# PaddlePaddle/PaddleNLP

Hardware: NVIDIA H100
Metric: tokens/sec Llama-3.2-3B seq4096 bf16 pretrain step (global, all GPUs) (higher is better)
Workload: dtype bf16

## Files before the change

paddlenlp_b200/csrc/abi.cu:

```cuda
#include <string.h>

#include <mutex>

#include "../../include/b200nlp.h"
#include "common.cuh"
#include "host_util.h"

namespace b200 {

static thread_local char tls_err[512] = "";

void set_last_error(const char* fmt, ...) {
  va_list ap;
  va_start(ap, fmt);
  vsnprintf(tls_err, sizeof(tls_err), fmt, ap);
  va_end(ap);
}
int fail_arg(const char* fmt, ...) {
  va_list ap;
  va_start(ap, fmt);
  vsnprintf(tls_err, sizeof(tls_err), fmt, ap);
  va_end(ap);
  return -1;
}
// ... 24 lines not shown
    cached[dev] = n > 0 ? n : 132;
  }
  return cached[dev];
}

typedef CUresult (*EncodeTiledFn)(CUtensorMap*, CUtensorMapDataType, cuuint32_t, void*, const cuuint64_t*,
                                  const cuuint64_t*, const cuuint32_t*, const cuuint32_t*, CUtensorMapInterleave,
                                  CUtensorMapSwizzle, CUtensorMapL2promotion, CUtensorMapFloatOOBfill);

static EncodeTiledFn get_encode_fn() {
  static EncodeTiledFn fn = nullptr;
  static std::once_flag once;
  std::call_once(once, []() {
    void* p = nullptr;
    cudaDriverEntryPointQueryResult qres;
    cudaError_t e = cudaGetDriverEntryPoint("cuTensorMapEncodeTiled", &p, cudaEnableDefault, &qres);
    if (e == cudaSuccess && qres == cudaDriverEntryPointSuccess) fn = reinterpret_cast<EncodeTiledFn>(p);
  });
  return fn;
}

static int encode_tmap(CUtensorMap* out, CUtensorMapDataType dtype, const void* base, int rank, const uint64_t* dims,
                       const uint64_t* strides, const uint32_t* box);

int encode_tmap_bf16(CUtensorMap* out, const void* base, int rank, const uint64_t* dims, const uint64_t* strides,
                     const uint32_t* box) {
  return encode_tmap(out, CU_TENSOR_MAP_DATA_TYPE_BFLOAT16, base, rank, dims, strides, box);
}
int encode_tmap_f32(CUtensorMap* out, const void* base, int rank, const uint64_t* dims, const uint64_t* strides,
                    const uint32_t* box) {
  return encode_tmap(out, CU_TENSOR_MAP_DATA_TYPE_FLOAT32, base, rank, dims, strides, box);
}

static int encode_tmap(CUtensorMap* out, CUtensorMapDataType dtype, const void* base, int rank, const uint64_t* dims,
                       const uint64_t* strides, const uint32_t* box) {
  EncodeTiledFn fn = get_encode_fn();
  if (!fn) return fail_arg("cuTensorMapEncodeTiled entry point unavailable (no CUDA driver?)");
  cuuint64_t gdim[5];
  cuuint64_t gstr[5];
  cuuint32_t bdim[5];
  cuuint32_t estr[5];
  for (int i = 0; i < rank; ++i) {
    gdim[i] = dims[i];
    bdim[i] = box[i];
    estr[i] = 1;
    if (i < rank - 1) gstr[i] = strides[i];
  }
  if ((reinterpret_cast<uintptr_t>(base) & 15) != 0) return fail_arg("tensor map base %p not 16-byte aligned", base);
  for (int i = 0; i < rank - 1; ++i)
    if (gstr[i] % 16 != 0) return fail_arg("tensor map stride %llu not a multiple of 16 bytes", (unsigned long long)gstr[i]);
  CUresult r = fn(out, dtype, static_cast<cuuint32_t>(rank), const_cast<void*>(base), gdim,
                  gstr, bdim, estr, CU_TENSOR_MAP_INTERLEAVE_NONE, CU_TENSOR_MAP_SWIZZLE_128B,
                  CU_TENSOR_MAP_L2_PROMOTION_L2_256B, CU_TENSOR_MAP_FLOAT_OOB_FILL_NONE);
  if (r != CUDA_SUCCESS)
    return fail_arg("cuTensorMapEncodeTiled failed (CUresult %d) rank=%d dims=[%llu,%llu] box=[%u,%u]", (int)r, rank,
                    (unsigned long long)dims[0], (unsigned long long)(rank > 1 ? dims[1] : 0), box[0],
                    rank > 1 ? box[1] : 0);
  return 0;
}

}

extern "C" {

const char* b200_last_error(void) { return b200::tls_err; }

// ... 36 lines not shown
```

paddlenlp_b200/csrc/common.cuh:

```cuda
#pragma once
#include <cuda.h>
#include <cuda_bf16.h>
#include <cuda_runtime.h>
#include <stdint.h>
#include <stdio.h>

namespace b200 {

typedef __nv_bfloat16 bf16;

__device__ __forceinline__ uint32_t smem_u32(const void* p) {
  return static_cast<uint32_t>(__cvta_generic_to_shared(p));
}
__device__ __forceinline__ void named_bar_sync(uint32_t id, uint32_t nthreads) {
  asm volatile("bar.sync %0, %1;" ::"r"(id), "r"(nthreads) : "memory");
}

__device__ __forceinline__ void pdl_wait() { asm volatile("griddepcontrol.wait;" ::: "memory"); }
__device__ __forceinline__ void pdl_launch_dependents() { asm volatile("griddepcontrol.launch_dependents;" ::: "memory"); }

__device__ __forceinline__ void mbar_init(uint64_t* bar, uint32_t count) {
  asm volatile("mbarrier.init.shared::cta.b64 [%0], %1;" ::"r"(smem_u32(bar)), "r"(count) : "memory");
}
__device__ __forceinline__ void fence_mbar_init() {
  asm volatile("fence.mbarrier_init.release.cluster;" ::: "memory");
}
__device__ __forceinline__ void fence_proxy_async_smem() {
  asm volatile("fence.proxy.async.shared::cta;" ::: "memory");
}
__device__ __forceinline__ void mbar_arrive_expect_tx(uint64_t* bar, uint32_t bytes) {
  asm volatile("mbarrier.arrive.expect_tx.shared::cta.b64 _, [%0], %1;" ::"r"(smem_u32(bar)), "r"(bytes)
               : "memory");
}
__device__ __forceinline__ void mbar_arrive(uint64_t* bar) {
  asm volatile("mbarrier.arrive.shared::cta.b64 _, [%0];" ::"r"(smem_u32(bar)) : "memory");
}
__device__ __forceinline__ bool mbar_try_wait(uint64_t* bar, uint32_t parity) {
  uint32_t ok;
  asm volatile(
      "{\n\t.reg .pred P;\n\t"
      "mbarrier.try_wait.parity.shared::cta.b64 P, [%1], %2;\n\t"
      "selp.u32 %0, 1, 0, P;\n\t}\n"
      : "=r"(ok)
      : "r"(smem_u32(bar)), "r"(parity)
      : "memory");
  return ok != 0;
}
__device__ __forceinline__ void mbar_wait(uint64_t* bar, uint32_t parity) {
// ... 60 lines not shown
  uint64_t d = 0;
  d |= static_cast<uint64_t>((saddr & 0x3FFFFu) >> 4);
  d |= static_cast<uint64_t>((lbo_bytes >> 4) & 0x3FFFu) << 16;
  d |= static_cast<uint64_t>((sbo_bytes >> 4) & 0x3FFFu) << 32;
  d |= static_cast<uint64_t>(1) << 62;
  return d;
}
__device__ __forceinline__ void wgmma_fence() { asm volatile("wgmma.fence.sync.aligned;" ::: "memory"); }
__device__ __forceinline__ void wgmma_commit() { asm volatile("wgmma.commit_group.sync.aligned;" ::: "memory"); }
template <int N>
__device__ __forceinline__ void wgmma_wait() { asm volatile("wgmma.wait_group.sync.aligned %0;" ::"n"(N) : "memory"); }
template <int R>
__device__ __forceinline__ void setmaxnreg_dec() { asm volatile("setmaxnreg.dec.sync.aligned.u32 %0;" ::"n"(R)); }
template <int R>
__device__ __forceinline__ void setmaxnreg_inc() { asm volatile("setmaxnreg.inc.sync.aligned.u32 %0;" ::"n"(R)); }

template <int TA, int TB>
__device__ __forceinline__ void wgmma_m64n256k16(float (&d)[128], uint64_t desc_a, uint64_t desc_b, uint32_t accumulate) {
  asm volatile(
      "{\n\t.reg .pred p;\n\tsetp.ne.b32 p, %130, 0;\n\t"
      "wgmma.mma_async.sync.aligned.m64n256k16.f32.bf16.bf16 "
      "{%0, %1, %2, %3, %4, %5, %6, %7, %8, %9, %10, %11, %12, %13, %14, %15, %16, %17, %18, %19, %20, %21, %22, %23, %24, %25, %26, %27, %28, %29, %30, %31, %32, %33, %34, %35, %36, %37, %38, %39, %40, %41, %42, %43, %44, %45, %46, %47, %48, %49, %50, %51, %52, %53, %54, %55, %56, %57, %58, %59, %60, %61, %62, %63, %64, %65, %66, %67, %68, %69, %70, %71, %72, %73, %74, %75, %76, %77, %78, %79, %80, %81, %82, %83, %84, %85, %86, %87, %88, %89, %90, %91, %92, %93, %94, %95, %96, %97, %98, %99, %100, %101, %102, %103, %104, %105, %106, %107, %108, %109, %110, %111, %112, %113, %114, %115, %116, %117, %118, %119, %120, %121, %122, %123, %124, %125, %126, %127}, %128, %129, p, 1, 1, %131, %132;\n\t}\n"
      : "+f"(d[0]), "+f"(d[1]), "+f"(d[2]), "+f"(d[3]), "+f"(d[4]), "+f"(d[5]), "+f"(d[6]), "+f"(d[7]), "+f"(d[8]), "+f"(d[9]), "+f"(d[10]), "+f"(d[11]), "+f"(d[12]), "+f"(d[13]), "+f"(d[14]), "+f"(d[15]), "+f"(d[16]), "+f"(d[17]), "+f"(d[18]), "+f"(d[19]), "+f"(d[20]), "+f"(d[21]), "+f"(d[22]), "+f"(d[23]), "+f"(d[24]), "+f"(d[25]), "+f"(d[26]), "+f"(d[27]), "+f"(d[28]), "+f"(d[29]), "+f"(d[30]), "+f"(d[31]), "+f"(d[32]), "+f"(d[33]), "+f"(d[34]), "+f"(d[35]), "+f"(d[36]), "+f"(d[37]), "+f"(d[38]), "+f"(d[39]), "+f"(d[40]), "+f"(d[41]), "+f"(d[42]), "+f"(d[43]), "+f"(d[44]), "+f"(d[45]), "+f"(d[46]), "+f"(d[47]), "+f"(d[48]), "+f"(d[49]), "+f"(d[50]), "+f"(d[51]), "+f"(d[52]), "+f"(d[53]), "+f"(d[54]), "+f"(d[55]), "+f"(d[56]), "+f"(d[57]), "+f"(d[58]), "+f"(d[59]), "+f"(d[60]), "+f"(d[61]), "+f"(d[62]), "+f"(d[63]), "+f"(d[64]), "+f"(d[65]), "+f"(d[66]), "+f"(d[67]), "+f"(d[68]), "+f"(d[69]), "+f"(d[70]), "+f"(d[71]), "+f"(d[72]), "+f"(d[73]), "+f"(d[74]), "+f"(d[75]), "+f"(d[76]), "+f"(d[77]), "+f"(d[78]), "+f"(d[79]), "+f"(d[80]), "+f"(d[81]), "+f"(d[82]), "+f"(d[83]), "+f"(d[84]), "+f"(d[85]), "+f"(d[86]), "+f"(d[87]), "+f"(d[88]), "+f"(d[89]), "+f"(d[90]), "+f"(d[91]), "+f"(d[92]), "+f"(d[93]), "+f"(d[94]), "+f"(d[95]), "+f"(d[96]), "+f"(d[97]), "+f"(d[98]), "+f"(d[99]), "+f"(d[100]), "+f"(d[101]), "+f"(d[102]), "+f"(d[103]), "+f"(d[104]), "+f"(d[105]), "+f"(d[106]), "+f"(d[107]), "+f"(d[108]), "+f"(d[109]), "+f"(d[110]), "+f"(d[111]), "+f"(d[112]), "+f"(d[113]), "+f"(d[114]), "+f"(d[115]), "+f"(d[116]), "+f"(d[117]), "+f"(d[118]), "+f"(d[119]), "+f"(d[120]), "+f"(d[121]), "+f"(d[122]), "+f"(d[123]), "+f"(d[124]), "+f"(d[125]), "+f"(d[126]), "+f"(d[127])
      : "l"(desc_a), "l"(desc_b), "r"(accumulate), "n"(TA), "n"(TB));
}
template <int TA, int TB>
__device__ __forceinline__ void wgmma_m64n64k16(float (&d)[32], uint64_t desc_a, uint64_t desc_b, uint32_t accumulate) {
  asm volatile(
      "{\n\t.reg .pred p;\n\tsetp.ne.b32 p, %34, 0;\n\t"
      "wgmma.mma_async.sync.aligned.m64n64k16.f32.bf16.bf16 "
      "{%0, %1, %2, %3, %4, %5, %6, %7, %8, %9, %10, %11, %12, %13, %14, %15, %16, %17, %18, %19, %20, %21, %22, %23, %24, %25, %26, %27, %28, %29, %30, %31}, %32, %33, p, 1, 1, %35, %36;\n\t}\n"
      : "+f"(d[0]), "+f"(d[1]), "+f"(d[2]), "+f"(d[3]), "+f"(d[4]), "+f"(d[5]), "+f"(d[6]), "+f"(d[7]), "+f"(d[8]), "+f"(d[9]), "+f"(d[10]), "+f"(d[11]), "+f"(d[12]), "+f"(d[13]), "+f"(d[14]), "+f"(d[15]), "+f"(d[16]), "+f"(d[17]), "+f"(d[18]), "+f"(d[19]), "+f"(d[20]), "+f"(d[21]), "+f"(d[22]), "+f"(d[23]), "+f"(d[24]), "+f"(d[25]), "+f"(d[26]), "+f"(d[27]), "+f"(d[28]), "+f"(d[29]), "+f"(d[30]), "+f"(d[31])
      : "l"(desc_a), "l"(desc_b), "r"(accumulate), "n"(TA), "n"(TB));
}
template <int TB>
__device__ __forceinline__ void wgmma_m64n128k16_rs(float (&d)[64], const uint32_t* a, uint64_t desc_b, uint32_t accumulate) {
  asm volatile(
      "{\n\t.reg .pred p;\n\tsetp.ne.b32 p, %69, 0;\n\t"
      "wgmma.mma_async.sync.aligned.m64n128k16.f32.bf16.bf16 "
      "{%0, %1, %2, %3, %4, %5, %6, %7, %8, %9, %10, %11, %12, %13, %14, %15, %16, %17, %18, %19, %20, %21, %22, %23, %24, %25, %26, %27, %28, %29, %30, %31, %32, %33, %34, %35, %36, %37, %38, %39, %40, %41, %42, %43, %44, %45, %46, %47, %48, %49, %50, %51, %52, %53, %54, %55, %56, %57, %58, %59, %60, %61, %62, %63}, {%64, %65, %66, %67}, %68, p, 1, 1, %70;\n\t}\n"
      : "+f"(d[0]), "+f"(d[1]), "+f"(d[2]), "+f"(d[3]), "+f"(d[4]), "+f"(d[5]), "+f"(d[6]), "+f"(d[7]), "+f"(d[8]), "+f"(d[9]), "+f"(d[10]), "+f"(d[11]), "+f"(d[12]), "+f"(d[13]), "+f"(d[14]), "+f"(d[15]), "+f"(d[16]), "+f"(d[17]), "+f"(d[18]), "+f"(d[19]), "+f"(d[20]), "+f"(d[21]), "+f"(d[22]), "+f"(d[23]), "+f"(d[24]), "+f"(d[25]), "+f"(d[26]), "+f"(d[27]), "+f"(d[28]), "+f"(d[29]), "+f"(d[30]), "+f"(d[31]), "+f"(d[32]), "+f"(d[33]), "+f"(d[34]), "+f"(d[35]), "+f"(d[36]), "+f"(d[37]), "+f"(d[38]), "+f"(d[39]), "+f"(d[40]), "+f"(d[41]), "+f"(d[42]), "+f"(d[43]), "+f"(d[44]), "+f"(d[45]), "+f"(d[46]), "+f"(d[47]), "+f"(d[48]), "+f"(d[49]), "+f"(d[50]), "+f"(d[51]), "+f"(d[52]), "+f"(d[53]), "+f"(d[54]), "+f"(d[55]), "+f"(d[56]), "+f"(d[57]), "+f"(d[58]), "+f"(d[59]), "+f"(d[60]), "+f"(d[61]), "+f"(d[62]), "+f"(d[63])
      : "r"(a[0]), "r"(a[1]), "r"(a[2]), "r"(a[3]), "l"(desc_b), "r"(accumulate), "n"(TB));
}

__device__ __forceinline__ void mma_bf16_16816(float (&c)[4], const uint32_t (&a)[4], uint32_t b0, uint32_t b1) {
  asm volatile(
      "mma.sync.aligned.m16n8k16.row.col.f32.bf16.bf16.f32 {%0, %1, %2, %3}, {%4, %5, %6, %7}, {%8, %9}, "
      "{%0, %1, %2, %3};"
      : "+f"(c[0]), "+f"(c[1]), "+f"(c[2]), "+f"(c[3])
      : "r"(a[0]), "r"(a[1]), "r"(a[2]), "r"(a[3]), "r"(b0), "r"(b1));
}
__device__ __forceinline__ void ldsm_x4(uint32_t saddr, uint32_t (&r)[4]) {
  asm volatile("ldmatrix.sync.aligned.m8n8.x4.shared.b16 {%0, %1, %2, %3}, [%4];"
               : "=r"(r[0]), "=r"(r[1]), "=r"(r[2]), "=r"(r[3])
               : "r"(saddr));
}
__device__ __forceinline__ void ldsm_x4_t(uint32_t saddr, uint32_t (&r)[4]) {
  asm volatile("ldmatrix.sync.aligned.m8n8.x4.trans.shared.b16 {%0, %1, %2, %3}, [%4];"
               : "=r"(r[0]), "=r"(r[1]), "=r"(r[2]), "=r"(r[3])
               : "r"(saddr));
}
__device__ __forceinline__ void cp_async_16(uint32_t saddr, const void* gptr, uint32_t src_bytes) {
  asm volatile("cp.async.cg.shared.global [%0], [%1], 16, %2;" ::"r"(saddr), "l"(gptr), "r"(src_bytes) : "memory");
}
__device__ __forceinline__ void cp_async_commit() { asm volatile("cp.async.commit_group;" ::: "memory"); }
template <int N>
// ... 80 lines not shown
```

paddlenlp_b200/csrc/fa_bwd.cu:

```cuda
#include <climits>

#include "../../include/b200nlp.h"
#include "common.cuh"
#include "host_util.h"

namespace b200 {
namespace fab {

constexpr int D = 128;
constexpr int BKV = 64;
constexpr int NUM_THREADS = 256;

struct Params {
  const bf16 *q, *k, *v, *dout;
  int64_t ldq, ldk, ldv, lddo;
  int S, B, nh, kvh, Spad;
  float scale, scale_log2;
  const float* lse2;
  const float* delta;
  const int* mask_start;
  float* dq_acc;
  float* dk_acc;
  float* dv_acc;
};
// ... 214 lines not shown
    o.z = pack_bf16x2(b.x, b.y); o.w = pack_bf16x2(b.z, b.w);
    *(reinterpret_cast<uint4*>(dq + t * lddq) + c) = o;
  }
}

namespace wg {
constexpr int BKV = 128;
constexpr int BQ = 64;
constexpr int STAGES = 2;
constexpr int NUM_THREADS = 256;
constexpr int KV_BYTES = BKV * D * 2;
constexpr int QT_BYTES = BQ * D * 2;
constexpr int STAGE_BYTES = 2 * QT_BYTES + 2 * BQ * 4;
constexpr int STAGE_STRIDE = 33 * 1024;
constexpr int DS_BYTES = BKV * BQ * 2;
constexpr int DQ_BYTES = BQ * 64 * 4;
constexpr int OFF_K = 0, OFF_V = KV_BYTES, OFF_RING = 2 * KV_BYTES;
constexpr int OFF_DS = OFF_RING + STAGES * STAGE_STRIDE;
constexpr int OFF_DQ = OFF_DS + 2 * DS_BYTES;
constexpr int OFF_BAR = OFF_DQ + 2 * DQ_BYTES;
constexpr int SMEM_BYTES = OFF_BAR + 64 + 1024;
static_assert(SMEM_BYTES <= 227 * 1024, "fa_bwd_wgmma: shared memory");
static_assert(STAGE_BYTES <= STAGE_STRIDE && 64 * D * 4 <= STAGE_STRIDE && 64 * D * 4 <= 2 * DS_BYTES && 64 * D * 4 <= 2 * DQ_BYTES,
              "fa_bwd_wgmma: shared-memory layout");

struct Params {
  int S, nh, kvh, Spad;
  float scale, scale_log2;
  const float* lse2;
  const float* delta;
  const int* mask_start;
};

template <int N>
__device__ __forceinline__ void reg_fence(float (&r)[N]) {
#pragma unroll
  for (int i = 0; i < N; ++i) asm volatile("" : "+f"(r[i])::"memory");
}

template <int NJ>
__device__ __forceinline__ void stage_f32(uint32_t base, const float (&acc)[4 * NJ], int wi, int lane) {
  const int g = lane >> 2, tq = lane & 3;
#pragma unroll
  for (int i = 0; i < 2; ++i) {
    const int row = wi * 16 + g + 8 * i;
#pragma unroll
    for (int j = 0; j < NJ; ++j) {
      const int chunk = (j & 3) * 2 + (tq >> 1);
      const uint32_t a = base + (j >> 2) * (64 * 128) + row * 128 + ((chunk ^ (row & 7)) << 4) + (tq & 1) * 8;
      asm volatile("st.shared.v2.f32 [%0], {%1, %2};" ::"r"(a), "f"(acc[4 * j + 2 * i]), "f"(acc[4 * j + 2 * i + 1]) : "memory");
    }
  }
}

template <bool MASK>
__global__ void __launch_bounds__(NUM_THREADS, 1)
fa_bwd_wgmma_kernel(const __grid_constant__ CUtensorMap tmQ, const __grid_constant__ CUtensorMap tmK,
                    const __grid_constant__ CUtensorMap tmV, const __grid_constant__ CUtensorMap tmdO,
                    const __grid_constant__ CUtensorMap tmdQ, const __grid_constant__ CUtensorMap tmdK,
                    const __grid_constant__ CUtensorMap tmdV, const Params p) {
  extern __shared__ uint8_t smem_raw[];
  uint8_t* smem = reinterpret_cast<uint8_t*>((reinterpret_cast<uintptr_t>(smem_raw) + 1023) & ~uintptr_t(1023));
  uint64_t* full_bar = reinterpret_cast<uint64_t*>(smem + OFF_BAR);
  uint64_t* empty_bar = full_bar + STAGES;
  uint64_t* kv_bar = empty_bar + STAGES;

  const int head = static_cast<int>(blockIdx.x) % p.nh, batch = static_cast<int>(blockIdx.x) / p.nh;
  const int kv_head = head / (p.nh / p.kvh);
  const int kv0 = static_cast<int>(blockIdx.y) * BKV;
  int q_lo = kv0 / BQ, q_hi = (p.S + BQ - 1) / BQ;
  if constexpr (MASK) {
    const int last = __ldg(p.mask_start + static_cast<size_t>(batch) * p.S + min(kv0 + BKV - 1, p.S - 1));
// ... 144 lines not shown
    mbar_arrive(&empty_bar[st]);
    uint8_t* sdq = smem + OFF_DQ + cw * DQ_BYTES;
    if (leader) tma_store_wait_read<0>();
    named_bar_sync(2 + cw, 128);
    stage_f32<8>(smem_u32(sdq), dq, wi, lane);
    fence_proxy_async_smem();
    named_bar_sync(2 + cw, 128);
    if (leader) {
      tma_reduce_add_4d(&tmdQ, sdq, cw * 64, head, q0, batch);
      tma_reduce_add_4d(&tmdQ, sdq + DQ_BYTES / 2, cw * 64 + 32, head, q0, batch);
      tma_store_commit();
    }
  }

  if (leader) tma_store_wait_read<0>();
  named_bar_sync(1, 256);
  uint8_t* sdk = smem + OFF_RING + cw * STAGE_STRIDE;
  uint8_t* sdv = smem + (cw == 0 ? OFF_DS : OFF_DQ);
  stage_f32<16>(smem_u32(sdk), dk, wi, lane);
  stage_f32<16>(smem_u32(sdv), dv, wi, lane);
  fence_proxy_async_smem();
  named_bar_sync(2 + cw, 128);
  if (leader) {
#pragma unroll
    for (int b = 0; b < 4; ++b) {
      tma_reduce_add_4d(&tmdK, sdk + b * (64 * 128), b * 32, kv_head, kv0 + cw * 64, batch);
      tma_reduce_add_4d(&tmdV, sdv + b * (64 * 128), b * 32, kv_head, kv0 + cw * 64, batch);
    }
    tma_store_commit();
    tma_store_wait<0>();
  }
}

static int make_bf16_map(CUtensorMap* tm, const void* base, int64_t B, int64_t S, int64_t heads, int64_t ld, uint32_t rows) {
  const uint64_t dims[4] = {128, static_cast<uint64_t>(heads), static_cast<uint64_t>(S), static_cast<uint64_t>(B)};
  const uint64_t strides[3] = {256, static_cast<uint64_t>(ld) * 2, static_cast<uint64_t>(S * ld) * 2};
  const uint32_t box[4] = {64, 1, rows, 1};
  return encode_tmap_bf16(tm, base, 4, dims, strides, box);
}
static int make_f32_map(CUtensorMap* tm, float* base, int64_t B, int64_t S, int64_t heads) {
  const uint64_t dims[4] = {128, static_cast<uint64_t>(heads), static_cast<uint64_t>(S), static_cast<uint64_t>(B)};
  const uint64_t strides[3] = {512, static_cast<uint64_t>(heads) * 512, static_cast<uint64_t>(S * heads) * 512};
  const uint32_t box[4] = {32, 1, 64, 1};
  return encode_tmap_f32(tm, base, 4, dims, strides, box);
}

template <bool MASK>
static int launch(const CUtensorMap (&tm)[7], const Params& p, int B, cudaStream_t stream) {
  auto kern = fa_bwd_wgmma_kernel<MASK>;
  static bool attr_set = false;
  if (!attr_set) {
    cudaError_t e = cudaFuncSetAttribute(kern, cudaFuncAttributeMaxDynamicSharedMemorySize, SMEM_BYTES);
    if (e != cudaSuccess) {
      set_last_error("fa_bwd_wgmma smem attr: %s", cudaGetErrorString(e));
      return static_cast<int>(e);
    }
    attr_set = true;
  }
  const dim3 grid(static_cast<unsigned>(p.nh * B), static_cast<unsigned>((p.S + BKV - 1) / BKV));
  kern<<<grid, NUM_THREADS, SMEM_BYTES, stream>>>(tm[0], tm[1], tm[2], tm[3], tm[4], tm[5], tm[6], p);
  return check_launch("fa_bwd_wgmma");
}
}

template <int BQ, bool MASK>
static int launch(const Params& p, cudaStream_t stream) {
  constexpr int SMEM = 2 * BKV * 256 + 2 * BQ * 256 + 2 * BQ * 128 + 2 * BQ * 4;
  static bool attr_set = false;
  if (!attr_set) {
    cudaError_t e = cudaFuncSetAttribute(fa_bwd_kernel<BQ, MASK>, cudaFuncAttributeMaxDynamicSharedMemorySize, SMEM);
    if (e != cudaSuccess) {
      set_last_error("fa_bwd smem attr: %s", cudaGetErrorString(e));
// ... 47 lines not shown
  float* dk_acc = dq_acc + B * S * num_heads * 128;
  float* dv_acc = dk_acc + B * S * num_kv_heads * 128;
  float* lse2 = dq_acc + 3 * B * S * num_heads * 128;
  float* delta = lse2 + B * num_heads * Spad;
  cudaError_t e = cudaMemsetAsync(dq_acc, 0, static_cast<size_t>(B) * S * (num_heads + 2 * num_kv_heads) * 128 * 4, stream);
  if (e != cudaSuccess) {
    set_last_error("fa_bwd memset: %s", cudaGetErrorString(e));
    return static_cast<int>(e);
  }
  {
    const int64_t rows = B * Spad * num_heads;
    const int64_t threads = rows * 16;
    fa_bwd_delta_kernel<<<static_cast<unsigned>((threads + 255) / 256), 256, 0, stream>>>(
        static_cast<const bf16*>(o), static_cast<const bf16*>(dout), lse, lse2, delta, (int)B, (int)S, (int)Spad, (int)num_heads,
        ldo, lddo);
    int rc = check_launch("fa_bwd(delta)");
    if (rc) return rc;
  }
  int rc;
  if (fa_bwd_impl() == 1) {
    Params p;
    p.q = static_cast<const bf16*>(q); p.k = static_cast<const bf16*>(k); p.v = static_cast<const bf16*>(v);
    p.dout = static_cast<const bf16*>(dout);
    p.ldq = ldq; p.ldk = ldk; p.ldv = ldv; p.lddo = lddo;
    p.S = (int)S; p.B = (int)B; p.nh = (int)num_heads; p.kvh = (int)num_kv_heads; p.Spad = (int)Spad;
    p.scale = softmax_scale;
    p.scale_log2 = softmax_scale * 1.4426950408889634f;
    p.lse2 = lse2; p.delta = delta;
    p.mask_start = mask_start_rows;
    p.dq_acc = dq_acc; p.dk_acc = dk_acc; p.dv_acc = dv_acc;
    rc = mask_start_rows ? launch<64, true>(p, stream) : launch<64, false>(p, stream);
  } else {
    CUtensorMap tm[7];
    if ((rc = wg::make_bf16_map(&tm[0], q, B, S, num_heads, ldq, wg::BQ)) != 0) return rc;
    if ((rc = wg::make_bf16_map(&tm[1], k, B, S, num_kv_heads, ldk, wg::BKV)) != 0) return rc;
    if ((rc = wg::make_bf16_map(&tm[2], v, B, S, num_kv_heads, ldv, wg::BKV)) != 0) return rc;
    if ((rc = wg::make_bf16_map(&tm[3], dout, B, S, num_heads, lddo, wg::BQ)) != 0) return rc;
    if ((rc = wg::make_f32_map(&tm[4], dq_acc, B, S, num_heads)) != 0) return rc;
    if ((rc = wg::make_f32_map(&tm[5], dk_acc, B, S, num_kv_heads)) != 0) return rc;
    if ((rc = wg::make_f32_map(&tm[6], dv_acc, B, S, num_kv_heads)) != 0) return rc;
    wg::Params p;
    p.S = (int)S; p.nh = (int)num_heads; p.kvh = (int)num_kv_heads; p.Spad = (int)Spad;
    p.scale = softmax_scale;
    p.scale_log2 = softmax_scale * 1.4426950408889634f;
    p.lse2 = lse2; p.delta = delta;
    p.mask_start = mask_start_rows;
    rc = mask_start_rows ? wg::launch<true>(tm, p, (int)B, stream) : wg::launch<false>(tm, p, (int)B, stream);
  }
  if (rc) return rc;
  {
    const int64_t tokens = B * S;
    const int width = static_cast<int>(num_heads * 128);
    const int64_t total = tokens * (width / 8);
    int64_t blocks = (total + 255) / 256;
    const int64_t cap = static_cast<int64_t>(sm_count()) * 16;
    if (blocks > cap) blocks = cap;
    fa_bwd_dq_finish_kernel<<<static_cast<unsigned>(blocks), 256, 0, stream>>>(dq_acc, static_cast<bf16*>(dq), tokens,
                                                                              width, lddq);
    if ((rc = check_launch("fa_bwd(dq finish)")) != 0) return rc;
    const int kvw = static_cast<int>(num_kv_heads * 128);
    int64_t kblocks = (tokens * (kvw / 8) + 255) / 256;
    if (kblocks > cap) kblocks = cap;
    fa_bwd_dq_finish_kernel<<<static_cast<unsigned>(kblocks), 256, 0, stream>>>(dk_acc, static_cast<bf16*>(dk), tokens, kvw,
                                                                               lddk);
    if ((rc = check_launch("fa_bwd(dk finish)")) != 0) return rc;
    fa_bwd_dq_finish_kernel<<<static_cast<unsigned>(kblocks), 256, 0, stream>>>(dv_acc, static_cast<bf16*>(dv), tokens, kvw,
                                                                               lddv);
    rc = check_launch("fa_bwd(dv finish)");
  }
  return rc;
// ... 2 lines not shown
```

paddlenlp_b200/csrc/fa_fwd.cu:

```cuda
#include "../../include/b200nlp.h"
#include "common.cuh"
#include "host_util.h"

namespace b200 {
namespace fa {

constexpr int D = 128;
constexpr int BKV = 64;
constexpr int KV_TILE_BYTES = BKV * D * 2;

enum Mode { DENSE = 0, MASK = 1, PAGED = 2 };

struct Params {
  const bf16* q;
  const bf16* k;
  const bf16* v;
  bf16* o;
  float* lse;
  int64_t ldq, ldk, ldv, ldo;
  int S, B, nh, kvh;
  float scale_log2;
  const int* mask_start;
  const int* cu_q;
  const int* seq_dec;
  const int* seq_this;
  const int* seq_enc;
  const int* block_tables;
  int max_blocks, block_size;
};

__device__ __forceinline__ uint32_t swz(int row, int chunk) { return static_cast<uint32_t>(row * 256 + ((chunk ^ (row & 7)) << 4)); }

template <int NW, int MODE>
__global__ void __launch_bounds__(NW * 32, 1) fa_fwd_kernel(const Params p) {
  constexpr int BQ = 16 * NW;
  extern __shared__ __align__(128) uint8_t smem[];
  const uint32_t sQ = smem_u32(smem);
  const uint32_t sK = sQ + BQ * 256;
  const uint32_t sV = sK + 2 * KV_TILE_BYTES;

  const int warp = threadIdx.x >> 5, lane = threadIdx.x & 31;
  const int head = blockIdx.y, batch = blockIdx.z;
  const int kv_head = head / (p.nh / p.kvh);
  int n_rows = p.S, pos0 = 0, tok0 = batch * p.S;
  if constexpr (MODE == PAGED) {
    n_rows = p.seq_this[batch];
    if (n_rows <= 0 || (n_rows == 1 && p.seq_enc[batch] <= 0)) return;
    pos0 = p.seq_dec[batch];
    tok0 = p.cu_q[batch];
  }
  const int qt = (n_rows + BQ - 1) / BQ - 1 - static_cast<int>(blockIdx.x);
  if (qt < 0) return;
  const int q0 = qt * BQ;
  const int kv_total = pos0 + n_rows;
  const int kv_end = pos0 + min(q0 + BQ, n_rows);
  const int n_kv = (kv_end + BKV - 1) / BKV;
  int j_lo = 0;
  if constexpr (MODE == MASK) {
    const int* ms = p.mask_start + static_cast<size_t>(batch) * p.S;
    while (j_lo < n_kv - 1 && __ldg(ms + min(j_lo * BKV + BKV - 1, p.S - 1)) <= q0) ++j_lo;
  }

  auto kv_row = [&](const bf16* base, int64_t ld, int c) -> const bf16* {
    if constexpr (MODE == PAGED) {
      const int page = __ldg(p.block_tables + static_cast<size_t>(batch) * p.max_blocks + c / p.block_size);
      return base + ((static_cast<size_t>(page) * p.kvh + kv_head) * p.block_size + c % p.block_size) * D;
// ... 95 lines not shown
#pragma unroll
      for (int dt = 0; dt < 16; ++dt) { o[dt][2 * h] *= corr; o[dt][2 * h + 1] *= corr; }
    }
#pragma unroll
    for (int kc = 0; kc < 4; ++kc) {
#pragma unroll
      for (int dp = 0; dp < 8; ++dp) {
        uint32_t b[4];
        ldsm_x4_t(vb + swz(kc * 16 + (lane & 7) + ((lane >> 3) & 1) * 8, dp * 2 + (lane >> 4)), b);
        mma_bf16_16816(o[2 * dp], pa[kc], b[0], b[1]);
        mma_bf16_16816(o[2 * dp + 1], pa[kc], b[2], b[3]);
      }
    }
    __syncthreads();
  }
#pragma unroll
  for (int h = 0; h < 2; ++h) {
    float lt = l[h];
    lt += __shfl_xor_sync(0xffffffffu, lt, 1);
    lt += __shfl_xor_sync(0xffffffffu, lt, 2);
    const int r = row_a + 8 * h;
    if (r >= n_rows) continue;
    const float inv = 1.f / lt;
    bf16* orow = p.o + static_cast<size_t>(tok0 + r) * p.ldo + head * D;
#pragma unroll
    for (int dt = 0; dt < 16; ++dt)
      *reinterpret_cast<uint32_t*>(orow + dt * 8 + 2 * tq) = pack_bf16x2(o[dt][2 * h] * inv, o[dt][2 * h + 1] * inv);
    if constexpr (MODE != PAGED) {
      if (tq == 0) p.lse[(static_cast<size_t>(batch) * p.nh + head) * p.S + r] = (m[h] + log2f(lt)) * 0.6931471805599453f;
    }
  }
}

template <int NW, int MODE>
static int launch(const Params& p, int q_rows, cudaStream_t stream) {
  constexpr int SMEM = 16 * NW * 256 + 4 * KV_TILE_BYTES;
  static bool attr_set = false;
  if (!attr_set) {
    cudaError_t e = cudaFuncSetAttribute(fa_fwd_kernel<NW, MODE>, cudaFuncAttributeMaxDynamicSharedMemorySize, SMEM);
    if (e != cudaSuccess) {
      set_last_error("fa_fwd smem attr: %s", cudaGetErrorString(e));
      return static_cast<int>(e);
    }
    attr_set = true;
  }
  dim3 grid(static_cast<unsigned>((q_rows + 16 * NW - 1) / (16 * NW)), static_cast<unsigned>(p.nh), static_cast<unsigned>(p.B));
  fa_fwd_kernel<NW, MODE><<<grid, NW * 32, SMEM, stream>>>(p);
  return check_launch("fa_fwd");
}

}

int launch_fa_prefill_paged(const void* qkv, const void* key_cache, const void* value_cache, void* out, const int32_t* cu_seqlens_q,
                            const int32_t* seq_lens_encoder, const int32_t* seq_lens_decoder, const int32_t* seq_lens_this_time,
                            const int32_t* block_tables, int64_t B, int64_t token_num, int64_t max_q_len, int64_t num_heads,
                            int64_t num_kv_heads, int64_t num_blocks, int64_t block_size, int64_t max_blocks_per_seq, int64_t ldq,
                            int64_t ldo, float softmax_scale, cudaStream_t stream) {
  using namespace fa;
  (void)token_num; (void)num_blocks;
  Params p = {};
  p.q = static_cast<const bf16*>(qkv);
  p.k = static_cast<const bf16*>(key_cache);
  p.v = static_cast<const bf16*>(value_cache);
  p.o = static_cast<bf16*>(out);
  p.ldq = ldq; p.ldo = ldo;
  p.S = static_cast<int>(max_q_len); p.B = static_cast<int>(B); p.nh = static_cast<int>(num_heads);
  p.kvh = static_cast<int>(num_kv_heads);
  p.scale_log2 = softmax_scale * 1.4426950408889634f;
  p.cu_q = cu_seqlens_q; p.seq_dec = seq_lens_decoder; p.seq_this = seq_lens_this_time; p.seq_enc = seq_lens_encoder;
  p.block_tables = block_tables;
  p.max_blocks = static_cast<int>(max_blocks_per_seq); p.block_size = static_cast<int>(block_size);
  return launch<8, PAGED>(p, static_cast<int>(max_q_len), stream);
}

}

extern "C" int b200_fa_fwd(const void* q, const void* k, const void* v, void* o, float* lse, int64_t B, int64_t S,
                           int64_t num_heads, int64_t num_kv_heads, int64_t head_dim, int64_t ldq, int64_t ldk,
                           int64_t ldv, int64_t ldo, float softmax_scale, cudaStream_t stream) {
  return b200_fa_fwd_flashmask(q, k, v, o, lse, nullptr, B, S, num_heads, num_kv_heads, head_dim, ldq, ldk, ldv, ldo,
                               softmax_scale, stream);
}

extern "C" int b200_fa_fwd_flashmask(const void* q, const void* k, const void* v, void* o, float* lse,
                                     const int32_t* mask_start_rows, int64_t B, int64_t S, int64_t num_heads,
                                     int64_t num_kv_heads, int64_t head_dim, int64_t ldq, int64_t ldk, int64_t ldv,
                                     int64_t ldo, float softmax_scale, cudaStream_t stream) {
  using namespace b200;
  using namespace b200::fa;
  B200_CHECK_ARG(q && k && v && o && lse, "fa_fwd: null pointer");
  B200_CHECK_ARG(head_dim == 128, "fa_fwd: head_dim must be 128 (got %lld)", (long long)head_dim);
  B200_CHECK_ARG(B > 0 && S > 0 && num_heads > 0 && num_kv_heads > 0 && num_heads % num_kv_heads == 0,
                 "fa_fwd: bad shape B=%lld S=%lld nh=%lld kvh=%lld", (long long)B, (long long)S, (long long)num_heads,
                 (long long)num_kv_heads);
  B200_CHECK_ARG(ldq % 8 == 0 && ldk % 8 == 0 && ldv % 8 == 0 && ldo % 8 == 0, "fa_fwd: token strides must be multiples of 8");
  Params p = {};
  p.q = static_cast<const bf16*>(q);
  p.k = static_cast<const bf16*>(k);
  p.v = static_cast<const bf16*>(v);
  p.o = static_cast<bf16*>(o);
  p.lse = lse;
  p.ldq = ldq; p.ldk = ldk; p.ldv = ldv; p.ldo = ldo;
  p.S = static_cast<int>(S); p.B = static_cast<int>(B); p.nh = static_cast<int>(num_heads);
  p.kvh = static_cast<int>(num_kv_heads);
  p.scale_log2 = softmax_scale * 1.4426950408889634f;
  p.mask_start = mask_start_rows;
  const int rows = static_cast<int>(S);
  if (fa_fwd_impl() == 1)
    return mask_start_rows ? launch<4, MASK>(p, rows, stream) : launch<4, DENSE>(p, rows, stream);
  return mask_start_rows ? launch<8, MASK>(p, rows, stream) : launch<8, DENSE>(p, rows, stream);
}
```

paddlenlp_b200/csrc/host_util.h:

```cpp
#pragma once
#include <cuda.h>
#include <cuda_runtime.h>
#include <stdarg.h>
#include <stdint.h>
#include <stdio.h>

namespace b200 {

void set_last_error(const char* fmt, ...);
int fail_arg(const char* fmt, ...);
int check_launch(const char* what);

int sm_count();
int fa_fwd_impl();
int fa_bwd_impl();
int launch_fa_prefill_paged(const void* qkv, const void* key_cache, const void* value_cache, void* out, const int32_t* cu_seqlens_q,
                            const int32_t* seq_lens_encoder, const int32_t* seq_lens_decoder, const int32_t* seq_lens_this_time,
                            const int32_t* block_tables, int64_t B, int64_t token_num, int64_t max_q_len, int64_t num_heads,
                            int64_t num_kv_heads, int64_t num_blocks, int64_t block_size, int64_t max_blocks_per_seq, int64_t ldq,
                            int64_t ldo, float softmax_scale, cudaStream_t stream);
bool pdl_enabled();

template <typename... KArgs, typename... Args>
inline cudaError_t launch_pdl(void (*kern)(KArgs...), dim3 grid, dim3 block, size_t smem, cudaStream_t stream, Args... args) {
  cudaLaunchConfig_t cfg = {};
  cfg.gridDim = grid;
  cfg.blockDim = block;
  cfg.dynamicSmemBytes = smem;
  cfg.stream = stream;
  cudaLaunchAttribute attr[1];
  attr[0].id = cudaLaunchAttributeProgrammaticStreamSerialization;
  attr[0].val.programmaticStreamSerializationAllowed = 1;
  cfg.attrs = attr;
  cfg.numAttrs = pdl_enabled() ? 1 : 0;
  return cudaLaunchKernelEx(&cfg, kern, static_cast<KArgs>(args)...);
}

int encode_tmap_bf16(CUtensorMap* out, const void* base, int rank, const uint64_t* dims, const uint64_t* strides,
                     const uint32_t* box);
int encode_tmap_f32(CUtensorMap* out, const void* base, int rank, const uint64_t* dims, const uint64_t* strides,
                    const uint32_t* box);

}

#define B200_CHECK_ARG(cond, ...)                  \
  do {                                             \
    if (!(cond)) return b200::fail_arg(__VA_ARGS__); \
  } while (0)
```

Measured before the change: 20300.

## Add TMA+WGMMA flash-attention forward kernel with ping-pong warpgroups

Adds a Hopper forward attention kernel that loads Q/K/V tiles with TMA into a 6-stage mbarrier ring and computes QK^T and PV with wgmma. It is made the default forward path in place of the warp-level mma kernel. Two warpgroups alternate tensor-core issue via named barriers, so one group's softmax overlaps the other's GEMMs, and the PV GEMM of one tile is overlapped with the S GEMM of the next. Query tiles are scheduled heaviest-first for causal balance. The cost is more code and shared memory, plus an extra per-call tensor-map encode on the host. The legacy 4-warp option is dropped.

After: 20830, median of 6. +2.6%, better.

```diff
diff --git a/paddlenlp_b200/csrc/abi.cu b/paddlenlp_b200/csrc/abi.cu
--- a/paddlenlp_b200/csrc/abi.cu
+++ b/paddlenlp_b200/csrc/abi.cu
@@ -80,6 +80,13 @@
   return encode_tmap(out, CU_TENSOR_MAP_DATA_TYPE_FLOAT32, base, rank, dims, strides, box);
 }
 
+int make_bf16_map(CUtensorMap* tm, const void* base, int64_t B, int64_t S, int64_t heads, int64_t ld, uint32_t rows) {
+  const uint64_t dims[4] = {128, static_cast<uint64_t>(heads), static_cast<uint64_t>(S), static_cast<uint64_t>(B)};
+  const uint64_t strides[3] = {256, static_cast<uint64_t>(ld) * 2, static_cast<uint64_t>(S * ld) * 2};
+  const uint32_t box[4] = {64, 1, rows, 1};
+  return encode_tmap_bf16(tm, base, 4, dims, strides, box);
+}
+
 static int encode_tmap(CUtensorMap* out, CUtensorMapDataType dtype, const void* base, int rank, const uint64_t* dims,
                        const uint64_t* strides, const uint32_t* box) {
   EncodeTiledFn fn = get_encode_fn();
diff --git a/paddlenlp_b200/csrc/common.cuh b/paddlenlp_b200/csrc/common.cuh
--- a/paddlenlp_b200/csrc/common.cuh
+++ b/paddlenlp_b200/csrc/common.cuh
@@ -14,6 +14,9 @@
 }
 __device__ __forceinline__ void named_bar_sync(uint32_t id, uint32_t nthreads) {
   asm volatile("bar.sync %0, %1;" ::"r"(id), "r"(nthreads) : "memory");
+}
+__device__ __forceinline__ void named_bar_arrive(uint32_t id, uint32_t nthreads) {
+  asm volatile("bar.arrive %0, %1;" ::"r"(id), "r"(nthreads) : "memory");
 }
 
 __device__ __forceinline__ void pdl_wait() { asm volatile("griddepcontrol.wait;" ::: "memory"); }
@@ -140,6 +143,11 @@
       "{%0, %1, %2, %3, %4, %5, %6, %7, %8, %9, %10, %11, %12, %13, %14, %15, %16, %17, %18, %19, %20, %21, %22, %23, %24, %25, %26, %27, %28, %29, %30, %31}, %32, %33, p, 1, 1, %35, %36;\n\t}\n"
       : "+f"(d[0]), "+f"(d[1]), "+f"(d[2]), "+f"(d[3]), "+f"(d[4]), "+f"(d[5]), "+f"(d[6]), "+f"(d[7]), "+f"(d[8]), "+f"(d[9]), "+f"(d[10]), "+f"(d[11]), "+f"(d[12]), "+f"(d[13]), "+f"(d[14]), "+f"(d[15]), "+f"(d[16]), "+f"(d[17]), "+f"(d[18]), "+f"(d[19]), "+f"(d[20]), "+f"(d[21]), "+f"(d[22]), "+f"(d[23]), "+f"(d[24]), "+f"(d[25]), "+f"(d[26]), "+f"(d[27]), "+f"(d[28]), "+f"(d[29]), "+f"(d[30]), "+f"(d[31])
       : "l"(desc_a), "l"(desc_b), "r"(accumulate), "n"(TA), "n"(TB));
+}
+template <int N>
+__device__ __forceinline__ void reg_fence(float (&r)[N]) {
+#pragma unroll
+  for (int i = 0; i < N; ++i) asm volatile("" : "+f"(r[i])::"memory");
 }
 template <int TB>
 __device__ __forceinline__ void wgmma_m64n128k16_rs(float (&d)[64], const uint32_t* a, uint64_t desc_b, uint32_t accumulate) {
diff --git a/paddlenlp_b200/csrc/fa_bwd.cu b/paddlenlp_b200/csrc/fa_bwd.cu
--- a/paddlenlp_b200/csrc/fa_bwd.cu
+++ b/paddlenlp_b200/csrc/fa_bwd.cu
@@ -270,12 +270,6 @@
   const int* mask_start;
 };
 
-template <int N>
-__device__ __forceinline__ void reg_fence(float (&r)[N]) {
-#pragma unroll
-  for (int i = 0; i < N; ++i) asm volatile("" : "+f"(r[i])::"memory");
-}
-
 template <int NJ>
 __device__ __forceinline__ void stage_f32(uint32_t base, const float (&acc)[4 * NJ], int wi, int lane) {
   const int g = lane >> 2, tq = lane & 3;
@@ -486,12 +480,6 @@
   }
 }
 
-static int make_bf16_map(CUtensorMap* tm, const void* base, int64_t B, int64_t S, int64_t heads, int64_t ld, uint32_t rows) {
-  const uint64_t dims[4] = {128, static_cast<uint64_t>(heads), static_cast<uint64_t>(S), static_cast<uint64_t>(B)};
-  const uint64_t strides[3] = {256, static_cast<uint64_t>(ld) * 2, static_cast<uint64_t>(S * ld) * 2};
-  const uint32_t box[4] = {64, 1, rows, 1};
-  return encode_tmap_bf16(tm, base, 4, dims, strides, box);
-}
 static int make_f32_map(CUtensorMap* tm, float* base, int64_t B, int64_t S, int64_t heads) {
   const uint64_t dims[4] = {128, static_cast<uint64_t>(heads), static_cast<uint64_t>(S), static_cast<uint64_t>(B)};
   const uint64_t strides[3] = {512, static_cast<uint64_t>(heads) * 512, static_cast<uint64_t>(S * heads) * 512};
@@ -605,10 +593,10 @@
     rc = mask_start_rows ? launch<64, true>(p, stream) : launch<64, false>(p, stream);
   } else {
     CUtensorMap tm[7];
-    if ((rc = wg::make_bf16_map(&tm[0], q, B, S, num_heads, ldq, wg::BQ)) != 0) return rc;
-    if ((rc = wg::make_bf16_map(&tm[1], k, B, S, num_kv_heads, ldk, wg::BKV)) != 0) return rc;
-    if ((rc = wg::make_bf16_map(&tm[2], v, B, S, num_kv_heads, ldv, wg::BKV)) != 0) return rc;
-    if ((rc = wg::make_bf16_map(&tm[3], dout, B, S, num_heads, lddo, wg::BQ)) != 0) return rc;
+    if ((rc = make_bf16_map(&tm[0], q, B, S, num_heads, ldq, wg::BQ)) != 0) return rc;
+    if ((rc = make_bf16_map(&tm[1], k, B, S, num_kv_heads, ldk, wg::BKV)) != 0) return rc;
+    if ((rc = make_bf16_map(&tm[2], v, B, S, num_kv_heads, ldv, wg::BKV)) != 0) return rc;
+    if ((rc = make_bf16_map(&tm[3], dout, B, S, num_heads, lddo, wg::BQ)) != 0) return rc;
     if ((rc = wg::make_f32_map(&tm[4], dq_acc, B, S, num_heads)) != 0) return rc;
     if ((rc = wg::make_f32_map(&tm[5], dk_acc, B, S, num_kv_heads)) != 0) return rc;
     if ((rc = wg::make_f32_map(&tm[6], dv_acc, B, S, num_kv_heads)) != 0) return rc;
diff --git a/paddlenlp_b200/csrc/fa_fwd.cu b/paddlenlp_b200/csrc/fa_fwd.cu
--- a/paddlenlp_b200/csrc/fa_fwd.cu
+++ b/paddlenlp_b200/csrc/fa_fwd.cu
@@ -1,3 +1,5 @@
+#include <climits>
+
 #include "../../include/b200nlp.h"
 #include "common.cuh"
 #include "host_util.h"
@@ -8,6 +10,7 @@
 constexpr int D = 128;
 constexpr int BKV = 64;
 constexpr int KV_TILE_BYTES = BKV * D * 2;
+constexpr int NW = 8;
 
 enum Mode { DENSE = 0, MASK = 1, PAGED = 2 };
 
@@ -31,7 +34,7 @@
 
 __device__ __forceinline__ uint32_t swz(int row, int chunk) { return static_cast<uint32_t>(row * 256 + ((chunk ^ (row & 7)) << 4)); }
 
-template <int NW, int MODE>
+template <int MODE>
 __global__ void __launch_bounds__(NW * 32, 1) fa_fwd_kernel(const Params p) {
   constexpr int BQ = 16 * NW;
   extern __shared__ __align__(128) uint8_t smem[];
@@ -193,12 +196,12 @@
   }
 }
 
-template <int NW, int MODE>
+template <int MODE>
 static int launch(const Params& p, int q_rows, cudaStream_t stream) {
   constexpr int SMEM = 16 * NW * 256 + 4 * KV_TILE_BYTES;
   static bool attr_set = false;
   if (!attr_set) {
-    cudaError_t e = cudaFuncSetAttribute(fa_fwd_kernel<NW, MODE>, cudaFuncAttributeMaxDynamicSharedMemorySize, SMEM);
+    cudaError_t e = cudaFuncSetAttribute(fa_fwd_kernel<MODE>, cudaFuncAttributeMaxDynamicSharedMemorySize, SMEM);
     if (e != cudaSuccess) {
       set_last_error("fa_fwd smem attr: %s", cudaGetErrorString(e));
       return static_cast<int>(e);
@@ -206,8 +209,231 @@
     attr_set = true;
   }
   dim3 grid(static_cast<unsigned>((q_rows + 16 * NW - 1) / (16 * NW)), static_cast<unsigned>(p.nh), static_cast<unsigned>(p.B));
-  fa_fwd_kernel<NW, MODE><<<grid, NW * 32, SMEM, stream>>>(p);
+  fa_fwd_kernel<MODE><<<grid, NW * 32, SMEM, stream>>>(p);
   return check_launch("fa_fwd");
+}
+
+namespace wg {
+constexpr int BQ = 128;
+constexpr int BKV = 64;
+constexpr int STAGES = 6;
+constexpr int NUM_THREADS = 256;
+constexpr int Q_BYTES = BQ * D * 2;
+constexpr int Q_HALF = Q_BYTES / 2;
+constexpr int KV_BYTES = BKV * D * 2;
+constexpr int KV_HALF = KV_BYTES / 2;
+constexpr int OFF_Q = 0, OFF_RING = Q_BYTES;
+constexpr int OFF_BAR = OFF_RING + STAGES * 2 * KV_BYTES;
+constexpr int SMEM_BYTES = OFF_BAR + 64 + 1024;
+static_assert(SMEM_BYTES <= 227 * 1024, "fa_fwd_wgmma: shared memory");
+constexpr uint32_t BAR_TURN = 1;
+
+struct Params {
+  bf16* o;
+  float* lse;
+  int64_t ldo;
+  int S, nh, kvh;
+  float scale_log2;
+  const int* mask_start;
+};
+
+template <bool MASK>
+__global__ void __launch_bounds__(NUM_THREADS, 1)
+fa_fwd_wgmma_kernel(const __grid_constant__ CUtensorMap tmQ, const __grid_constant__ CUtensorMap tmK,
+                    const __grid_constant__ CUtensorMap tmV, const Params p) {
+  extern __shared__ uint8_t smem_raw[];
+  uint8_t* smem = reinterpret_cast<uint8_t*>((reinterpret_cast<uintptr_t>(smem_raw) + 1023) & ~uintptr_t(1023));
+  uint64_t* full_bar = reinterpret_cast<uint64_t*>(smem + OFF_BAR);
+  uint64_t* empty_bar = full_bar + STAGES;
+  uint64_t* q_bar = empty_bar + STAGES;
+
+  const int head = static_cast<int>(blockIdx.x) % p.nh, batch = static_cast<int>(blockIdx.x) / p.nh;
+  const int kv_head = head / (p.nh / p.kvh);
+  const int q0 = ((p.S + BQ - 1) / BQ - 1 - static_cast<int>(blockIdx.y)) * BQ;
+  const int n_kv = (min(q0 + BQ, p.S) + BKV - 1) / BKV;
+  const int* ms = MASK ? p.mask_start + static_cast<size_t>(batch) * p.S : nullptr;
+  int j_lo = 0;
+  if constexpr (MASK) {
+    while (j_lo < n_kv - 1 && __ldg(ms + min(j_lo * BKV + BKV - 1, p.S - 1)) <= q0) ++j_lo;
+  }
+  if (threadIdx.x == 0) {
+    tma_prefetch_desc(&tmQ); tma_prefetch_desc(&tmK); tma_prefetch_desc(&tmV);
+    for (int i = 0; i < STAGES; ++i) {
+      mbar_init(&full_bar[i], 1);
+      mbar_init(&empty_bar[i], 256);
+    }
+    mbar_init(q_bar, 1);
+    fence_mbar_init();
+  }
+  __syncthreads();
+
+  const int n_tiles = n_kv - j_lo;
+  auto load_kv = [&](int t) {
+    const int st = t % STAGES;
+    uint8_t* sk = smem + OFF_RING + st * 2 * KV_BYTES;
+    mbar_arrive_expect_tx(&full_bar[st], 2 * KV_BYTES);
+    for (int h = 0; h < 2; ++h) {
+      tma_load_4d(&tmK, &full_bar[st], sk + h * KV_HALF, h * 64, kv_head, (j_lo + t) * BKV, batch);
+      tma_load_4d(&tmV, &full_bar[st], sk + KV_BYTES + h * KV_HALF, h * 64, kv_head, (j_lo + t) * BKV, batch);
+    }
+  };
+  if (threadIdx.x == 0) {
+    mbar_arrive_expect_tx(q_bar, Q_BYTES);
+    for (int h = 0; h < 2; ++h) tma_load_4d(&tmQ, q_bar, smem + OFF_Q + h * Q_HALF, h * 64, head, q0, batch);
+    for (int t = 0; t < STAGES && t < n_tiles; ++t) load_kv(t);
+  }
+
+  const int cw = threadIdx.x >> 7;
+  const int wi = (threadIdx.x >> 5) & 3, lane = threadIdx.x & 31, g = lane >> 2, tq = lane & 3;
+  const int row0 = q0 + cw * 64 + wi * 16 + g;
+  const uint32_t sQ = smem_u32(smem) + OFF_Q + cw * 64 * 128, sRing = smem_u32(smem) + OFF_RING;
+  float o[64], s[32];
+#pragma unroll
+  for (int i = 0; i < 64; ++i) o[i] = 0.f;
+  float m[2] = {-INFINITY, -INFINITY}, l[2] = {0.f, 0.f}, corr[2];
+  uint32_t pa[16];
+
+  auto issue_s = [&](int st) {
+    const uint32_t sK = sRing + st * 2 * KV_BYTES;
+#pragma unroll
+    for (int kk = 0; kk < 8; ++kk) {
+      const uint32_t qo = (kk >> 2) * Q_HALF + (kk & 3) * 32, ko = (kk >> 2) * KV_HALF + (kk & 3) * 32;
+      wgmma_m64n64k16<0, 0>(s, wgmma_desc_sw128(sQ + qo, 16, 1024), wgmma_desc_sw128(sK + ko, 16, 1024), kk > 0 ? 1u : 0u);
+    }
+    wgmma_commit();
+  };
+  auto issue_pv = [&](int st) {
+    const uint32_t sV = sRing + st * 2 * KV_BYTES + KV_BYTES;
+#pragma unroll
+    for (int k = 0; k < 4; ++k) wgmma_m64n128k16_rs<1>(o, pa + 4 * k, wgmma_desc_sw128(sV + k * 2048, KV_HALF, 1024), 1u);
+    wgmma_commit();
+  };
+  auto softmax = [&](int j) {
+    const int kv0 = j * BKV;
+    const bool need_causal = kv0 + BKV - 1 > q0 + cw * 64 + wi * 16;
+    bool need_mask = false;
+    if constexpr (MASK) need_mask = __ldg(ms + kv0) <= q0 + BQ - 1;
+    if (need_causal || need_mask) {
+#pragma unroll
+      for (int jj = 0; jj < 8; ++jj)
+#pragma unroll
+        for (int e = 0; e < 2; ++e) {
+          const int c = kv0 + 8 * jj + 2 * tq + e;
+          int lim = INT_MAX;
+          if constexpr (MASK) {
+            if (c < p.S) lim = __ldg(ms + c);
+          }
+#pragma unroll
+          for (int i = 0; i < 2; ++i) {
+            const int r = row0 + 8 * i;
+            if (c > r || r >= lim) s[4 * jj + 2 * i + e] = -INFINITY;
+          }
+        }
+    }
+#pragma unroll
+    for (int i = 0; i < 2; ++i) {
+      float mx = -INFINITY;
+#pragma unroll
+      for (int jj = 0; jj < 8; ++jj) mx = fmaxf(mx, fmaxf(s[4 * jj + 2 * i], s[4 * jj + 2 * i + 1]));
+      mx = fmaxf(mx, __shfl_xor_sync(0xffffffffu, mx, 1));
+      mx = fmaxf(mx, __shfl_xor_sync(0xffffffffu, mx, 2));
+      const float m_new = fmaxf(m[i], mx * p.scale_log2);
+      corr[i] = (m[i] == -INFINITY) ? 0.f : fast_exp2(m[i] - m_new);
+      m[i] = m_new;
+      const float neg_m = (m_new == -INFINITY) ? 0.f : -m_new;
+      float rs = 0.f;
+#pragma unroll
+      for (int jj = 0; jj < 8; ++jj) {
+        float& x0 = s[4 * jj + 2 * i];
+        float& x1 = s[4 * jj + 2 * i + 1];
+        x0 = fast_exp2(fmaf(x0, p.scale_log2, neg_m));
+        x1 = fast_exp2(fmaf(x1, p.scale_log2, neg_m));
+        rs += x0 + x1;
+      }
+      l[i] = l[i] * corr[i] + rs;
+    }
+  };
+  auto pack_p = [&]() {
+#pragma unroll
+    for (int t = 0; t < 16; ++t) pa[t] = pack_bf16x2(s[2 * t], s[2 * t + 1]);
+  };
+
+  if (cw == 1) named_bar_arrive(BAR_TURN, 256);
+  mbar_wait_nocall(q_bar, 0);
+  mbar_wait_nocall(&full_bar[0], 0);
+  named_bar_sync(BAR_TURN + cw, 256);
+  wgmma_fence();
+  issue_s(0);
+  named_bar_arrive(BAR_TURN + (cw ^ 1), 256);
+  wgmma_wait<0>();
+  reg_fence(s);
+  softmax(j_lo);
+  pack_p();
+  for (int j = j_lo + 1, it = 1; j < n_kv; ++j, ++it) {
+    const int st = it % STAGES, pst = (it - 1) % STAGES;
+    mbar_wait_nocall(&full_bar[st], (it / STAGES) & 1);
+    named_bar_sync(BAR_TURN + cw, 256);
+    wgmma_fence();
+    issue_s(st);
+    issue_pv(pst);
+    named_bar_arrive(BAR_TURN + (cw ^ 1), 256);
+    wgmma_wait<1>();
+    reg_fence(s);
+    softmax(j);
+    wgmma_wait<0>();
+    reg_fence(o);
+    mbar_arrive(&empty_bar[pst]);
+    if (threadIdx.x == 128 && it - 1 + STAGES < n_tiles) {
+      mbar_wait_nocall(&empty_bar[pst], ((it - 1) / STAGES) & 1);
+      load_kv(it - 1 + STAGES);
+    }
+#pragma unroll
+    for (int jj = 0; jj < 16; ++jj)
+#pragma unroll
+      for (int i = 0; i < 2; ++i) {
+        o[4 * jj + 2 * i] *= corr[i];
+        o[4 * jj + 2 * i + 1] *= corr[i];
+      }
+    pack_p();
+  }
+  named_bar_sync(BAR_TURN + cw, 256);
+  wgmma_fence();
+  issue_pv((n_kv - 1 - j_lo) % STAGES);
+  if (cw == 0) named_bar_arrive(BAR_TURN + 1, 256);
+  wgmma_wait<0>();
+  reg_fence(o);
+#pragma unroll
+  for (int i = 0; i < 2; ++i) {
+    float lt = l[i];
+    lt += __shfl_xor_sync(0xffffffffu, lt, 1);
+    lt += __shfl_xor_sync(0xffffffffu, lt, 2);
+    const int r = row0 + 8 * i;
+    if (r >= p.S) continue;
+    const float inv = 1.f / lt;
+    bf16* orow = p.o + (static_cast<size_t>(batch) * p.S + r) * p.ldo + head * D;
+#pragma unroll
+    for (int jj = 0; jj < 16; ++jj)
+      *reinterpret_cast<uint32_t*>(orow + 8 * jj + 2 * tq) = pack_bf16x2(o[4 * jj + 2 * i] * inv, o[4 * jj + 2 * i + 1] * inv);
+    if (tq == 0) p.lse[(static_cast<size_t>(batch) * p.nh + head) * p.S + r] = (m[i] + log2f(lt)) * 0.6931471805599453f;
+  }
+}
+
+template <bool MASK>
+static int launch(const CUtensorMap (&tm)[3], const Params& p, int B, cudaStream_t stream) {
+  auto kern = fa_fwd_wgmma_kernel<MASK>;
+  static bool attr_set = false;
+  if (!attr_set) {
+    cudaError_t e = cudaFuncSetAttribute(kern, cudaFuncAttributeMaxDynamicSharedMemorySize, SMEM_BYTES);
+    if (e != cudaSuccess) {
+      set_last_error("fa_fwd_wgmma smem attr: %s", cudaGetErrorString(e));
+      return static_cast<int>(e);
+    }
+    attr_set = true;
+  }
+  const dim3 grid(static_cast<unsigned>(p.nh * B), static_cast<unsigned>((p.S + BQ - 1) / BQ));
+  kern<<<grid, NUM_THREADS, SMEM_BYTES, stream>>>(tm[0], tm[1], tm[2], p);
+  return check_launch("fa_fwd_wgmma");
+}
 }
 
 }
@@ -231,7 +457,7 @@
   p.cu_q = cu_seqlens_q; p.seq_dec = seq_lens_decoder; p.seq_this = seq_lens_this_time; p.seq_enc = seq_lens_encoder;
   p.block_tables = block_tables;
   p.max_blocks = static_cast<int>(max_blocks_per_seq); p.block_size = static_cast<int>(block_size);
-  return launch<8, PAGED>(p, static_cast<int>(max_q_len), stream);
+  return launch<PAGED>(p, static_cast<int>(max_q_len), stream);
 }
 
 }
@@ -255,6 +481,27 @@
                  "fa_fwd: bad shape B=%lld S=%lld nh=%lld kvh=%lld", (long long)B, (long long)S, (long long)num_heads,
                  (long long)num_kv_heads);
   B200_CHECK_ARG(ldq % 8 == 0 && ldk % 8 == 0 && ldv % 8 == 0 && ldo % 8 == 0, "fa_fwd: token strides must be multiples of 8");
+  {
+    const void* ptrs[4] = {q, k, v, o};
+    const char* names[4] = {"q", "k", "v", "o"};
+    for (int i = 0; i < 4; ++i)
+      B200_CHECK_ARG((reinterpret_cast<uintptr_t>(ptrs[i]) & 15) == 0, "fa_fwd: %s must be 16-byte aligned (got %p)", names[i], ptrs[i]);
+  }
+  if (fa_fwd_impl() == 2) {
+    CUtensorMap tm[3];
+    int rc;
+    if ((rc = make_bf16_map(&tm[0], q, B, S, num_heads, ldq, wg::BQ)) != 0) return rc;
+    if ((rc = make_bf16_map(&tm[1], k, B, S, num_kv_heads, ldk, wg::BKV)) != 0) return rc;
+    if ((rc = make_bf16_map(&tm[2], v, B, S, num_kv_heads, ldv, wg::BKV)) != 0) return rc;
+    wg::Params p;
+    p.o = static_cast<bf16*>(o);
+    p.lse = lse;
+    p.ldo = ldo;
+    p.S = static_cast<int>(S); p.nh = static_cast<int>(num_heads); p.kvh = static_cast<int>(num_kv_heads);
+    p.scale_log2 = softmax_scale * 1.4426950408889634f;
+    p.mask_start = mask_start_rows;
+    return mask_start_rows ? wg::launch<true>(tm, p, static_cast<int>(B), stream) : wg::launch<false>(tm, p, static_cast<int>(B), stream);
+  }
   Params p = {};
   p.q = static_cast<const bf16*>(q);
   p.k = static_cast<const bf16*>(k);
@@ -267,7 +514,5 @@
   p.scale_log2 = softmax_scale * 1.4426950408889634f;
   p.mask_start = mask_start_rows;
   const int rows = static_cast<int>(S);
-  if (fa_fwd_impl() == 1)
-    return mask_start_rows ? launch<4, MASK>(p, rows, stream) : launch<4, DENSE>(p, rows, stream);
-  return mask_start_rows ? launch<8, MASK>(p, rows, stream) : launch<8, DENSE>(p, rows, stream);
-}
+  return mask_start_rows ? launch<MASK>(p, rows, stream) : launch<DENSE>(p, rows, stream);
+}
diff --git a/paddlenlp_b200/csrc/host_util.h b/paddlenlp_b200/csrc/host_util.h
--- a/paddlenlp_b200/csrc/host_util.h
+++ b/paddlenlp_b200/csrc/host_util.h
@@ -40,6 +40,7 @@
                      const uint32_t* box);
 int encode_tmap_f32(CUtensorMap* out, const void* base, int rank, const uint64_t* dims, const uint64_t* strides,
                     const uint32_t* box);
+int make_bf16_map(CUtensorMap* tm, const void* base, int64_t B, int64_t S, int64_t heads, int64_t ld, uint32_t rows);
 
 }
 
```
